# 10XGenomics/rust-pseudoaligner

Measured on AMD Instinct MI355X. Metric: reads/sec pseudoaligned (whole node) on synthetic 150bp reads, higher is better.
Workload: dtype u64; 1 GPU; config3: ~202k-transcript synthetic GENCODE-scale index (K=24), error-free 150bp reads; read_len=150, k=24, transcripts=201914, kmers=103866252, index_bytes=4833106924

## Files before the change

### rust-pseudoaligner_amd/csrc/map_pool.hip

```cpp
#include <hip/hip_runtime.h>

#include "kernels.hpp"
#include "lane_steps.hpp"
#include "kernel_utils.hpp"

#ifndef PA_FILL
#define PA_FILL 1
#endif
#ifndef PA_COOP_MIN
#define PA_COOP_MIN 2u
#endif
#ifndef PA_REFILL_ALIGN
#define PA_REFILL_ALIGN 1u
#endif
#ifndef PA_RARE_MIN
#define PA_RARE_MIN 16u
#endif

#ifdef PA_ISA_MARKS
#define PA_MARK(name) asm volatile("; PA_MARK " name ::: "memory")
#else
#define PA_MARK(name)
#endif

namespace pa {
namespace {

typedef __attribute__((address_space(3))) uint64_t* lds_u64;
typedef __attribute__((address_space(3))) uint32_t* lds_u32;
typedef __attribute__((address_space(3))) uint8_t* lds_u8;
typedef __attribute__((address_space(3))) uint16_t* lds_u16;
typedef __attribute__((address_space(3))) unsigned long long* lds_u64w;
typedef uint32_t u32x4 __attribute__((ext_vector_type(4)));
typedef __attribute__((address_space(3))) u32x4* lds_v4;
typedef __attribute__((address_space(1))) u32x4* glb_v4w;
typedef __attribute__((address_space(1))) const u32x4* glb_v4;
typedef __attribute__((address_space(1))) uint32_t* glb_u32w;
typedef __attribute__((address_space(1))) const uint32_t* glb_u32;
typedef __attribute__((address_space(1))) unsigned long long* glb_u64w;
__device__ __forceinline__ void store_result(glb_v4w dst, u32x4 v) {
    if (PA_NT & 2) __builtin_nontemporal_store(v, dst);
    else *dst = v;
}

typedef __attribute__((address_space(4))) const MapParams* karg_ptr;

__device__ __forceinline__ DevIndexView view_of(karg_ptr p) {
    DevIndexView v;
    v.table = p->ix.table; v.nbuckets = p->ix.nbuckets; v.blobs = p->ix.blobs; v.ledge = p->ix.ledge;
    v.seg_g = p->ix.seg_g; v.seg_nid = p->ix.seg_nid; v.ec = p->ix.ec; v.class_ref = p->ix.class_ref; v.class_len = p->ix.class_len;
    v.wtable = p->ix.wtable; v.wbuckets = p->ix.wbuckets; v.kmask = p->ix.kmask; v.kmask_hi = p->ix.kmask_hi; v.k = p->ix.k; v.num_nodes = p->ix.num_nodes; v.num_classes = p->ix.num_classes; v.num_segs = p->ix.num_segs; v.stream_nt = p->ix.stream_nt; v.bitmap_min = p->ix.bitmap_min; v.bitmap_words = p->ix.bitmap_words; v.dict_pairs = p->ix.dict_pairs;
    return v;
}

static_assert(ST_NSTAT == ST_COUNT + 4, "kernels.hpp");
constexpr uint32_t ST_DUAL = ST_COUNT;
constexpr uint32_t POOL_FIXED = 960;
constexpr uint32_t POOL_MAX_SLOTS = 128;
constexpr uint32_t LIST_ROW_HDR = 12;

__device__ __forceinline__ uint32_t rank_in(uint64_t m) { return __builtin_amdgcn_mbcnt_hi((uint32_t)(m >> 32), __builtin_amdgcn_mbcnt_lo((uint32_t)m, 0u)); }

__device__ __forceinline__ uint64_t shfl64(uint64_t v, uint32_t src) {
    return ((uint64_t)(uint32_t)__shfl((int)(v >> 32), (int)src, 64) << 32) | (uint32_t)__shfl((int)v, (int)src, 64);
}

__device__ __forceinline__ uint64_t arena_alloc(uint32_t cnt_alloc, uint32_t lane, karg_ptr p, lds_u64w chunk) {
    const uint32_t incl = wave_incl_scan(cnt_alloc);
    const uint32_t total = (uint32_t)__builtin_amdgcn_readlane((int)incl, 63);
    asm volatile("" ::: "memory");
    unsigned long long chunk_cur = chunk[0];
    if (total > 0) {
        if (chunk_cur + total > chunk[1]) {
            const unsigned long long want = total > PA_ARENA_CHUNK ? total : PA_ARENA_CHUNK;
            unsigned long long base = 0;
            if (lane == 0) base = atomicAdd(p->arena_top, want);
            base = ((unsigned long long)(uint32_t)__builtin_amdgcn_readfirstlane((int)(base >> 32)) << 32) | (uint32_t)__builtin_amdgcn_readfirstlane((int)base);
            chunk_cur = base;
            if (lane == 0) chunk[1] = base + want;
        }
        if (lane == 0) chunk[0] = chunk_cur + total;
    }
    asm volatile("" ::: "memory");
    return chunk_cur + (incl - cnt_alloc);
}

constexpr uint32_t NO_KEY = 0xFFFFFFFFu;
__device__ __forceinline__ void append_keys(uint32_t key, uint32_t lane, karg_ptr p, lds_u32 kchunk) {
    const uint64_t m = __ballot(key != NO_KEY);
    if (m == 0) return;
    const uint32_t cnt = (uint32_t)__popcll(m);
    const glb_u32w keys = (glb_u32w)p->keys;
    asm volatile("" ::: "memory");
    const uint32_t cur = kchunk[0], room = kchunk[1] - cur;
    uint32_t nbase = 0;
    if (cnt > room) {
        if (lane == 0) {
            nbase = (uint32_t)atomicAdd(p->keys_top, (unsigned long long)PA_KEY_CHUNK);
            if ((uint64_t)nbase + PA_KEY_CHUNK > p->keys_cap) { atomicOr(p->status, PA_STATUS_SPILL_OVERFLOW); nbase = 0; }
        }
        nbase = (uint32_t)__builtin_amdgcn_readfirstlane((int)nbase);
    }
    const uint32_t r = rank_in(m);
    if (key != NO_KEY) keys[r < room ? cur + r : nbase + (r - room)] = key;
    if (lane == 0) {
        if (cnt > room) { kchunk[0] = nbase + (cnt - room); kchunk[1] = nbase + PA_KEY_CHUNK; }
        else kchunk[0] = cur + cnt;
    }
    asm volatile("" ::: "memory");
}

__device__ __forceinline__ void append_deferred(bool has, u32x4 e0, u32x4 e1, uint32_t lane, karg_ptr p, lds_u32 dchunk) {
    const uint64_t m = __ballot(has);
    if (m == 0) return;
    const uint32_t cnt = (uint32_t)__popcll(m);
    const glb_v4w out = (glb_v4w)p->defer;
    asm volatile("" ::: "memory");
    const uint32_t cur = dchunk[0], room = dchunk[1] - cur;
    uint32_t nbase = 0;
    if (cnt > room) {
        if (lane == 0) {
            nbase = (uint32_t)atomicAdd(p->defer_top, (unsigned long long)PA_DEFER_CHUNK);
            if ((uint64_t)nbase + PA_DEFER_CHUNK > p->defer_cap) { atomicOr(p->status, PA_STATUS_SPILL_OVERFLOW); nbase = 0; }
        }
        nbase = (uint32_t)__builtin_amdgcn_readfirstlane((int)nbase);
    }
    if (has) {
        const uint32_t r = rank_in(m);
        const uint64_t at = 2ull * (r < room ? cur + r : nbase + (r - room));
        out[at] = e0;
        out[at + 1] = e1;
    }
    if (lane == 0) {
        if (cnt > room) { dchunk[0] = nbase + (cnt - room); dchunk[1] = nbase + PA_DEFER_CHUNK; }
        else dchunk[0] = cur + cnt;
    }
    asm volatile("" ::: "memory");
}

__device__ __forceinline__ uint32_t list_hits(glb_u32 ec, uint32_t xref, uint32_t nch, uint32_t maxch, const uint32_t (&b)[8]) {
    const glb_v4 xrec = (glb_v4)(ec + 4ull * xref);
    uint32_t acc = 0;
    for (uint32_t c0 = 0; c0 < maxch; c0 += 4) {
        u32x4 w[4];
#pragma unroll
        for (uint32_t t = 0; t < 4; ++t) w[t] = xrec[c0 + t < nch ? c0 + t : 0];
#pragma unroll
        for (uint32_t t = 0; t < 4; ++t)
            if (c0 + t < nch) {
                const U4 ww{w[t].x, w[t].y, w[t].z, w[t].w};
                acc |= scan_words(ww, c0 + t == 0, b);
            }
    }
    return acc;
}

__device__ __forceinline__ uint32_t wave_max(uint32_t v) {
    for (uint32_t o = 32; o; o >>= 1) v = max(v, (uint32_t)__shfl_xor((int)v, (int)o, 64));
    return (uint32_t)__builtin_amdgcn_readfirstlane((int)v);
}

__device__ __forceinline__ void window_hits(glb_u32 ec, uint32_t xref, uint32_t len, bool act, uint32_t b1, uint32_t b2, uint32_t bitmap_min, uint32_t& m1, uint32_t& m2) {
    const bool bm = act && bitmap_min != 0 && len >= bitmap_min;
    uint32_t bw[4] = {0u, 0u, 0u, 0u};
    if (__ballot(bm)) {
        if (bm) {
            const glb_u32 bits = ec + class_bitmap(xref, len);
            bw[0] = bits[b1 >> 5]; bw[1] = bits[(b1 >> 5) + 1]; bw[2] = bits[b2 >> 5]; bw[3] = bits[(b2 >> 5) + 1];
        }
    }
    act = act && !bm;
    const glb_v4 rec = (glb_v4)(ec + 4ull * xref);
    const uint32_t nch = act ? (len + 4) >> 2 : 0u;
    uint32_t c[2] = {0u, 0u}, e[2] = {nch, 0u};
    const bool lng = act && len > 64;
    if (__ballot(lng)) {
        if (lng) {
            const glb_u32 ids = ec + 4ull * xref + 1;
#pragma unroll
            for (uint32_t r = 0; r < 2; ++r) {
                const uint32_t b = r ? b2 : b1;
                uint32_t lo = 0, hi = len;
                while (lo < hi) {
                    const uint32_t mid = (lo + hi) >> 1;
                    if (ids[mid] < b) lo = mid + 1; else hi = mid;
                }
                c[r] = (1 + lo) >> 2;
                e[r] = min(nch, ((1 + lo + CLASS_WINDOW - 1) >> 2) + 1);
            }
        }
    }
    m1 = m2 = 0;
#pragma unroll
    for (uint32_t r = 0; r < 2; ++r) {
        const uint32_t mx = wave_max(e[r] > c[r] ? e[r] - c[r] : 0u);
        for (uint32_t c0 = 0; c0 < mx; c0 += 4) {
            u32x4 w[4];
#pragma unroll
            for (uint32_t t = 0; t < 4; ++t) w[t] = rec[c[r] + c0 + t < e[r] ? c[r] + c0 + t : 0u];
#pragma unroll
            for (uint32_t t = 0; t < 4; ++t)
                if (c[r] + c0 + t < e[r]) {
                    const uint32_t v[4] = {w[t].x, w[t].y, w[t].z, w[t].w};
#pragma unroll
                    for (uint32_t i = 0; i < 4; ++i) {
                        if (i == 0 && c[r] + c0 + t == 0) continue;
                        const uint32_t d1 = v[i] - b1, d2 = v[i] - b2;
                        if (d1 < CLASS_WINDOW) m1 |= 1u << d1;
                        if (d2 < CLASS_WINDOW) m2 |= 1u << d2;
                    }
                }
        }
    }
    if (bm) {
        m1 = (uint32_t)((((uint64_t)bw[1] << 32) | bw[0]) >> (b1 & 31u));
        m2 = (uint32_t)((((uint64_t)bw[3] << 32) | bw[2]) >> (b2 & 31u));
    }
}

}

namespace narrow {
#define PA_K_WIDE 0
#include "map_pool_kernel.inc"
#undef PA_K_WIDE
}

namespace wide {
#define PA_K_WIDE 1
#include "map_pool_kernel.inc"
#undef PA_K_WIDE
}

size_t pool_slot_bytes(uint32_t wpr) {
    return wpr > PA_LDS_READ_WORDS ? (size_t)wide::SLOT_FIXED_BYTES : 8 * (size_t)wpr + narrow::SLOT_FIXED_BYTES;
}
size_t pool_fixed_bytes() { return POOL_FIXED; }
uint32_t pool_max_slots() { return POOL_MAX_SLOTS; }

size_t pool_lds_bytes(uint32_t wpr, uint32_t slots) {
    const size_t wave_bytes = (POOL_FIXED + (size_t)slots * pool_slot_bytes(wpr) + 15) & ~(size_t)15;
    return wave_bytes * (PA_MAP_BLOCK / 64);
}

template <class K>
static int launch_kernel(K kernel, const MapParams& p, uint32_t grid, size_t lds_bytes, hipStream_t stream) {
    if (lds_bytes > 48 * 1024) {
        const hipError_t e = hipFuncSetAttribute(reinterpret_cast<const void*>(kernel), hipFuncAttributeMaxDynamicSharedMemorySize, (int)lds_bytes);
        if (e != hipSuccess) return (int)e;
    }
    hipLaunchKernelGGL(kernel, dim3(grid), dim3(PA_MAP_BLOCK), lds_bytes, stream, p);
    return (int)hipGetLastError();
}

int launch_map_pool(const MapParams& p, uint32_t grid, size_t lds_bytes, hipStream_t stream) {
    const bool gread = p.wpr > PA_LDS_READ_WORDS;
    const bool pair = p.ix.dict_pairs != 0;
    if (gread && pair) return p.trace ? launch_kernel(&wide::pa_map_pool_kernel<true, true, false, false, false, true>, p, grid, lds_bytes, stream)
                                      : launch_kernel(&wide::pa_map_pool_kernel<false, true, false, false, false, true>, p, grid, lds_bytes, stream);
    if (gread) return p.trace ? launch_kernel(&wide::pa_map_pool_kernel<true, true, false, false>, p, grid, lds_bytes, stream)
                              : launch_kernel(&wide::pa_map_pool_kernel<false, true, false, false>, p, grid, lds_bytes, stream);
    if (p.trace) return pair ? launch_kernel(&narrow::pa_map_pool_kernel<true, false, false, false, false, true>, p, grid, lds_bytes, stream)
                             : launch_kernel(&narrow::pa_map_pool_kernel<true, false, false, false>, p, grid, lds_bytes, stream);
#ifdef PA_DEBUG_KNOBS
    if (p.dbg || p.ablate) return pair ? launch_kernel(&narrow::pa_map_pool_kernel<false, false, true, false, false, true>, p, grid, lds_bytes, stream)
                                       : launch_kernel(&narrow::pa_map_pool_kernel<false, false, true, false>, p, grid, lds_bytes, stream);
#endif
    if (p.ix.k > 32)
        return p.pool_slots == 128 ? launch_kernel(&narrow::pa_map_pool_kernel<false, false, false, true, true>, p, grid, lds_bytes, stream)
                                   : launch_kernel(&narrow::pa_map_pool_kernel<false, false, false, false, true>, p, grid, lds_bytes, stream);
    if (pair) return p.pool_slots == 128 ? launch_kernel(&narrow::pa_map_pool_kernel<false, false, false, true, false, true>, p, grid, lds_bytes, stream)
                                         : launch_kernel(&narrow::pa_map_pool_kernel<false, false, false, false, false, true>, p, grid, lds_bytes, stream);
    if (p.pool_slots == 128) return launch_kernel(&narrow::pa_map_pool_kernel<false, false, false, true>, p, grid, lds_bytes, stream);
    return launch_kernel(&narrow::pa_map_pool_kernel<false, false, false, false>, p, grid, lds_bytes, stream);
}

int pool_kernel_occupancy(size_t lds_bytes, int* blocks_per_cu) {
    return (int)hipOccupancyMaxActiveBlocksPerMultiprocessor(blocks_per_cu, reinterpret_cast<const void*>(&narrow::pa_map_pool_kernel<false, false, false, false>),
                                                             PA_MAP_BLOCK, lds_bytes);
}

}
```

### rust-pseudoaligner_amd/csrc/map_pool_kernel.inc

```
namespace {

template <bool TRACE>
__device__ __forceinline__ void trace_out(const Lane& s, bool mapped, uint32_t gslot, karg_ptr p) {
    if (!TRACE) return;
    const uint32_t spill_cap = p->spill_cap;
    const uint32_t nt = l_ntrace(s);
    const uint32_t nn = mapped ? (nt < spill_cap ? nt : spill_cap) : 0;
    ((glb_u32w)p->nodes_len)[s.rid] = mapped ? nt : 0;
    const glb_u32w tr = (glb_u32w)p->trace + (uint64_t)gslot * spill_cap;
    const glb_u32w out = (glb_u32w)p->nodes_out + (uint64_t)s.rid * spill_cap;
    for (uint32_t j = 0; j < nn; ++j) out[j] = tr[j];
}

template <bool TRACE>
__device__ __forceinline__ uint32_t emit_record(Lane& s, uint32_t cnt, uint32_t cnt_alloc, uint64_t my_off, uint32_t base_len,
                                                uint32_t base_colour, uint32_t gslot, karg_ptr p, bool& defer) {
    uint32_t colour = NO_CLASS, class_off = (uint32_t)my_off;
    bool novel = false;
    if (my_off + cnt_alloc > p->arena_cap) atomicOr(p->status, PA_STATUS_ARENA_FULL);
    if (cnt == base_len) {
        colour = base_colour;
        class_off = PA_CLASS_REF | base_colour;
    } else novel = cnt != 0;
    if (l_flags(s) & F_SPILL_OVERFLOW) atomicOr(p->status, PA_STATUS_SPILL_OVERFLOW);
    ((glb_v4w)p->results)[s.rid] = u32x4{l_cov(s), l_mism(s) | PA_MAPPED_BIT, class_off, cnt};
    trace_out<TRACE>(s, true, gslot, p);
    const glb_u32w colour_out = (glb_u32w)p->colour_out;
    if (novel && (p->keys != nullptr || colour_out != nullptr) && my_off + cnt_alloc <= p->arena_cap) {
        defer = true;
        s.lk = 0;
        return NO_KEY;
    }
    if (colour_out) colour_out[s.rid] = colour;
    s.lk = 0;
    const uint32_t num_classes = p->ix.num_classes;
    return cnt == 0 ? num_classes + 1 : colour == NO_CLASS ? num_classes : colour;
}

__device__ __forceinline__ uint32_t queue_of(Lane& s, uint32_t K) {
    uint32_t st = l_st(s);
    if (st == ST_ISECT) {
        const uint32_t fl = l_flags(s);
        if (!(fl & F_LISTS)) {
            const uint32_t todo = window_todo(s);
            if (todo == 2) { restart_lists(s, K); return ST_SEEK; }
            st = todo ? ST_F_MASK : ST_F_BITS;
        } else st = l_ncol(s) <= 3 ? ST_F_LIGHT : (fl & F_SMALL_BASE) ? ST_F_SCAN : ST_F_COOP;
        l_set_st(s, st);
    }
    return st == ST_NONE ? (uint32_t)ST_F_BITS : st;
}

template <bool GREAD>
__device__ __forceinline__ void refill_slot(Lane& s, uint64_t rid, uint32_t slot, karg_ptr p, lds_u64 rd, lds_u32 wc, uint32_t S, uint32_t wpr,
                                            uint32_t K) {
    const uint32_t* lens = p->lens;
    uint32_t L = lens ? lens[rid] : p->uniform_len;
    if (L > wpr * 32) L = wpr * 32;
    if (!GREAD) {
        const uint64_t* src = p->tiles + ((rid >> 6) * wpr) * 64 + (rid & 63);
        if (wpr == 5) {
            const bool nt = (PA_NT & 1) || p->ix.stream_nt;
            const uint64_t v0 = ld_stream(src, nt), v1 = ld_stream(src + 64, nt), v2 = ld_stream(src + 128, nt), v3 = ld_stream(src + 192, nt), v4 = ld_stream(src + 256, nt);
            rd[slot] = v0; rd[S + slot] = v1; rd[2 * S + slot] = v2; rd[3 * S + slot] = v3; rd[4 * S + slot] = v4;
        } else if (wpr == 4) {
            const bool nt = (PA_NT & 1) || p->ix.stream_nt;
            const uint64_t v0 = ld_stream(src, nt), v1 = ld_stream(src + 64, nt), v2 = ld_stream(src + 128, nt), v3 = ld_stream(src + 192, nt);
            rd[slot] = v0; rd[S + slot] = v1; rd[2 * S + slot] = v2; rd[3 * S + slot] = v3;
        } else
        for (uint32_t w0 = 0; w0 < wpr; w0 += 8) {
            uint64_t v[8];
#pragma unroll
            for (uint32_t i = 0; i < 8; ++i) v[i] = w0 + i < wpr ? PA_LD(1, src + (uint64_t)(w0 + i) * 64) : 0ull;
#pragma unroll
            for (uint32_t i = 0; i < 8; ++i)
                if (w0 + i < wpr) rd[(w0 + i) * S + slot] = v[i];
        }
    }
    lane_start(s, (uint32_t)rid, L, K);
    wc[2 * slot + 1] = (uint32_t)rid;
}

__device__ __forceinline__ void lane_load(Lane& s, lds_v4 stA, lds_v4 stB, lds_v4 stC, uint32_t slot) {
    const u32x4 a = stA[slot], b = stB[slot];
    s.lk = a.x; s.cm = a.y; s.h = a.z; s.of = a.w; s.rr = b.x; s.rm = b.y; s.ph = b.z; s.nc = b.w;
#if PA_K_WIDE
    const u32x4 c = stC[slot];
    s.xl = c.x; s.xm = c.y; s.xt = c.z;
#else
    (void)stC;
#endif
}
__device__ __forceinline__ void lane_store(const Lane& s, lds_v4 stA, lds_v4 stB, lds_v4 stC, uint32_t slot) {
    stA[slot] = u32x4{s.lk, s.cm, s.h, s.of};
    stB[slot] = u32x4{s.rr, s.rm, s.ph, s.nc};
#if PA_K_WIDE
    stC[slot] = u32x4{s.xl, s.xm, s.xt, 0u};
#else
    (void)stC;
#endif
}
constexpr uint32_t SLOT_FIXED_BYTES = 32 + 16 + 8 + (PA_K_WIDE ? 16 : 0);

}

#ifndef PA_MAP_MIN_BLOCKS
#define PA_MAP_MIN_BLOCKS 3
#endif
template <bool TRACE, bool GREAD, bool DBG, bool S128 = false, bool KBIG = false, bool PAIR = false>
__global__ __launch_bounds__(PA_MAP_BLOCK, PA_MAP_MIN_BLOCKS) void pa_map_pool_kernel(const MapParams p_arg) {
    karg_ptr kp = (karg_ptr)__builtin_amdgcn_kernarg_segment_ptr();
    (void)p_arg;
#define p (*kp)
#define PA_DBG (DBG && p.dbg)
#define PA_ABLATE(bit) (DBG && (p.ablate & (bit)))
    extern __shared__ __attribute__((aligned(16))) uint8_t smem[];
    const uint32_t lane = lane_id();
    const uint32_t wave_in_block = (uint32_t)__builtin_amdgcn_readfirstlane((int)(threadIdx.x >> 6));
    const uint32_t waves_per_block = PA_MAP_BLOCK / 64;
    const uint32_t wave = blockIdx.x * waves_per_block + wave_in_block;
    const uint32_t nwaves = gridDim.x * waves_per_block;
    const uint32_t S = S128 ? 128u : p.pool_slots, wpr = p.wpr;
    const uint32_t lwpr = GREAD ? 0u : wpr;

    const uint32_t wave_bytes = (POOL_FIXED + S * (8 * lwpr + SLOT_FIXED_BYTES) + 15) & ~15u;
    uint8_t* const wbase = smem + wave_in_block * wave_bytes;
    const lds_u64w chunk = (lds_u64w)wbase;
    const lds_u32 dbg = (lds_u32)(wbase + 16);
    const lds_u64w dbg_clk = (lds_u64w)(wbase + 16 + 8 * ST_NSTAT);
    const lds_u32 kchunk = (lds_u32)(wbase + 256);
    const lds_u32 dchunk = (lds_u32)(wbase + 264);
    const lds_u64 rd = (lds_u64)(wbase + POOL_FIXED);
    const lds_v4 stA = (lds_v4)(wbase + POOL_FIXED + 8 * lwpr * S);
    const lds_v4 stB = (lds_v4)(wbase + POOL_FIXED + (8 * lwpr + 16) * S);
    constexpr uint32_t XW = PA_K_WIDE ? 16u : 0u;
    const lds_v4 stC = (lds_v4)(wbase + POOL_FIXED + (8 * lwpr + 32) * S);
    const lds_v4 win = (lds_v4)(wbase + POOL_FIXED + (8 * lwpr + 32 + XW) * S);
    const lds_u32 wc = (lds_u32)(wbase + POOL_FIXED + (8 * lwpr + 48 + XW) * S);
    const lds_u8 sb = (lds_u8)(wbase + 768);
    const lds_u8 poplist = (lds_u8)(wbase + 896);
    if (lane < 64) ((lds_u32)wbase)[lane] = 0;
    if (lane < 4) kchunk[lane] = 0;
    ((lds_u16)sb)[lane] = (uint16_t)((lane < S ? (uint32_t)ST_EMPTY : 0xFFu) | ((lane + 64 < S ? (uint32_t)ST_EMPTY : 0xFFu) << 8));

    const uint32_t ntiles = (uint32_t)((p.n_reads + 63) >> 6);
    const uint32_t chunk_tiles = ntiles / (nwaves * 4) >= 16 ? 16u : ntiles / (nwaves * 4) >= 1 ? ntiles / (nwaves * 4) : 1u;
    uint64_t next = (uint64_t)wave * chunk_tiles << 6;
    uint64_t end = (uint64_t)(wave + 1) * chunk_tiles << 6;
    if (end > p.n_reads) end = p.n_reads;
    if (next > end) next = end;
    bool more = true;
    uint32_t seen = nwaves * chunk_tiles;

    const bool counting = p.keys != nullptr;

#define PA_CNT(t) ((uint32_t)__popcll(__ballot(st_lo == (t))) + (uint32_t)__popcll(__ballot(st_hi == (t))))
#define PA_POP(t, nn, out)                                                                         \
    {                                                                                              \
        const uint64_t m0_ = __ballot(st_lo == (t)), m1_ = __ballot(st_hi == (t));                 \
        const uint32_t r1_ = (uint32_t)__popcll(m0_) + rank_in(m1_);                               \
        if (st_lo == (t)) poplist[rank_in(m0_)] = (uint8_t)lane;                                   \
        if (st_hi == (t) && r1_ < 64) poplist[r1_] = (uint8_t)(lane + 64);                         \
        asm volatile("" ::: "memory");                                                             \
        out = lane < (nn) ? (uint32_t)poplist[lane] : 0u;                                          \
        asm volatile("" ::: "memory");                                                             \
    }

    for (;;) {
        PA_MARK("loop_top");
        asm volatile("" : "+s"(kp) : : "memory");
        const DevIndexView ix = view_of(kp);
        const glb_u32 ec = (glb_u32)ix.ec;
        const uint32_t K = ix.k, allowed = p.allowed, spill_cap = p.spill_cap;
        if (next == end && more) {
            const uint32_t share = (ntiles > seen ? ntiles - seen : 0u) / (2 * nwaves);
            const uint32_t take = share >= 16 ? 16u : share >= 2 ? share : 2u;
            uint32_t t0 = 0;
            if (lane == 0) t0 = atomicAdd(p.tile_ctr, take);
            t0 = (uint32_t)__builtin_amdgcn_readfirstlane((int)t0) + nwaves * chunk_tiles;
            seen = t0 + take;
            if (t0 >= ntiles) more = false;
            else {
                next = (uint64_t)t0 << 6;
                end = (uint64_t)(t0 + take) << 6;
                if (end > p.n_reads) end = p.n_reads;
            }
        }
        const uint32_t st2 = (uint32_t)((lds_u16)sb)[lane];
        const uint32_t st_lo = st2 & 0xFFu, st_hi = st2 >> 8;
        const uint64_t left = end - next;
        const uint32_t nempty = PA_CNT(ST_EMPTY);
        const uint32_t nrefill = (uint32_t)(left < (uint64_t)nempty ? left : (uint64_t)nempty);
        uint32_t best = 0, sel = ST_EMPTY;
        uint32_t bestn = 0;
#define PA_CONSIDER(t, c) { const uint32_t c_ = (c); if (best < 64 && c_ > best) { best = c_; bestn = c_; sel = (t); } }
#define PA_CONSIDER_RARE_MIN(t, c, mn) { const uint32_t c_ = (c), w_ = (PA_RARE_MIN && c_ >= (mn)) ? 64u + c_ : c_; \
                                         if (best < 64 && w_ > best) { best = w_; bestn = c_; sel = (t); } }
#define PA_CONSIDER_RARE(t, c) PA_CONSIDER_RARE_MIN(t, c, PA_RARE_MIN)
        constexpr uint32_t RARE = (1u << ST_LEFT) | (1u << ST_F_LIGHT) | (1u << ST_F_SCAN) | (1u << ST_F_COOP) | (1u << ST_F_MASK);
        const bool any_rare = __ballot((((RARE >> (st_lo & 31u)) | (RARE >> (st_hi & 31u))) & 1u) != 0) != 0;
        const uint32_t n_bits_q = PA_CNT(ST_F_BITS), n_seek_q = PA_CNT(ST_SEEK), n_fwd_q = PA_CNT(ST_FWD);
        if (any_rare) {
            PA_CONSIDER_RARE_MIN(ST_F_COOP, PA_CNT(ST_F_COOP), PA_COOP_MIN)
            PA_CONSIDER_RARE(ST_F_SCAN, PA_CNT(ST_F_SCAN))
            PA_CONSIDER_RARE(ST_F_LIGHT, PA_CNT(ST_F_LIGHT))
            PA_CONSIDER_RARE(ST_F_MASK, PA_CNT(ST_F_MASK))
            PA_CONSIDER(ST_F_BITS, n_bits_q)
            PA_CONSIDER(ST_FWD, n_fwd_q)
            PA_CONSIDER_RARE(ST_LEFT, PA_CNT(ST_LEFT))
            PA_CONSIDER(ST_SEEK, n_seek_q)
            PA_CONSIDER(ST_EMPTY, nrefill)
        } else {
            const uint32_t cb = min(n_bits_q, 64u), cf = min(n_fwd_q, 64u), cs = min(n_seek_q, 64u), ce = min(nrefill, 64u);
            best = max(max(cb, cf), max(cs, ce));
            sel = cb == best ? (uint32_t)ST_F_BITS : cf == best ? (uint32_t)ST_FWD : cs == best ? (uint32_t)ST_SEEK : (uint32_t)ST_EMPTY;
            bestn = cb == best ? n_bits_q : cf == best ? n_fwd_q : cs == best ? n_seek_q : nrefill;
        }
#undef PA_CONSIDER
#undef PA_CONSIDER_RARE
#undef PA_CONSIDER_RARE_MIN
        if (best == 0) break;
#ifndef PA_SEEK_MIN
#define PA_SEEK_MIN 32u
#endif
        const bool seek_ok = n_seek_q >= PA_SEEK_MIN || n_fwd_q < 24;
        const bool dual = (sel == ST_FWD || sel == ST_SEEK) && (K <= 32 || KBIG) && n_seek_q != 0 && n_fwd_q != 0 && seek_ok && !PA_ABLATE(4u);
        if (dual) sel = ST_FWD;
        uint32_t n_own = dual ? (n_fwd_q < 64 ? n_fwd_q : 64) : bestn < 64 ? bestn : 64;
        if (PA_REFILL_ALIGN > 1 && sel == ST_EMPTY && n_own >= PA_REFILL_ALIGN && (uint64_t)n_own < left) n_own &= ~(PA_REFILL_ALIGN - 1u);
        const uint32_t n_fill = (PA_FILL && sel == ST_F_BITS && left != 0) ? (64 - n_own < nempty ? 64 - n_own : nempty) : 0u;
        const uint32_t n = n_own + n_fill;
        const uint32_t n2 = dual ? (n_seek_q < 64 ? n_seek_q : 64) : 0u;
        if (PA_DBG && lane == 0) {
            dbg[dual ? ST_DUAL : sel] += 1;
            dbg[ST_NSTAT + (dual ? ST_DUAL : sel)] += n + n2;
        }
        const unsigned long long t_sec = PA_DBG ? __builtin_readcyclecounter() : 0ull;

        PA_MARK("picked");
        const bool active = lane < n;
        uint32_t slot, slot2 = 0;
        PA_POP(sel, n_own, slot)
        if (n_fill) {
            uint32_t eslot;
            PA_POP((uint32_t)ST_EMPTY, n_fill, eslot)
            const uint32_t mine = (uint32_t)__shfl((int)eslot, (int)((lane - n_own) & 63u), 64);
            if (lane >= n_own && active) slot = mine;
        }
        const bool active2 = lane < n2;
        if (dual) PA_POP((uint32_t)ST_SEEK, n2, slot2)
        const uint32_t gslot = wave * S + slot;
        Lane s;
        {
            lane_load(s, stA, stB, stC, slot);
            s.rid = wc[2 * slot + 1];
            if (n_fill && lane >= n_own) s.lk = 0;
        }
        const ReadRef rr = GREAD ? ReadRef{p.tiles + ((uint64_t)(s.rid >> 6) * wpr) * 64 + (s.rid & 63), 64u, wpr} : ReadRef{(const uint64_t*)(rd + slot), S, wpr, true};
        const glb_u32w row = (glb_u32w)p.spill + (uint64_t)gslot * spill_cap;
        const ColRef cols{(uint32_t*)&win[slot], (uint32_t*)(wc + 2 * slot), (uint32_t*)row, (uint32_t*)(row + 4), (uint32_t*)(row + 8),
                          (uint32_t*)(row + LIST_ROW_HDR), spill_cap - LIST_ROW_HDR, (uint32_t*)row,
                          TRACE ? (uint32_t*)((glb_u32w)p.trace + (uint64_t)gslot * spill_cap) : nullptr};

        uint32_t nq2 = 0xFFu;
        PA_MARK("popped");
        const unsigned long long t_pop = PA_DBG ? __builtin_readcyclecounter() : 0ull;
        if (sel == ST_EMPTY) {
            if (active) refill_slot<GREAD>(s, next + lane, slot, kp, rd, wc, S, wpr, K);
            next += n;
        } else if (sel == ST_SEEK) {
            if (active) {
                if (PAIR) seek_step_pair(s, ix, rr);
                else seek_step_slots(s, ix, rr);
            }
        } else if (sel == ST_FWD) {
            __builtin_amdgcn_s_waitcnt(0x0F70);
            Lane s2;
            {
#if PA_K_WIDE
                lane_load(s2, stA, stB, stC, slot2);
                if (!active2) l_zero(s2);
#else
                const u32x4 a = stA[slot2], b = stB[slot2];
                s2.lk = active2 ? a.x : 0u; s2.cm = active2 ? a.y : 0u; s2.h = active2 ? a.z : 0u; s2.of = active2 ? a.w : 0u;
                s2.rr = active2 ? b.x : 0u; s2.rm = active2 ? b.y : 0u; s2.ph = active2 ? b.z : 0u; s2.nc = active2 ? b.w : 0u;
#endif
                s2.rid = 0;
            }
            if (!active) l_zero(s);
            const uint32_t rid2 = GREAD && active2 ? wc[2 * slot2 + 1] : 0u;
            const ReadRef rr2 = GREAD ? ReadRef{p.tiles + ((uint64_t)(rid2 >> 6) * wpr) * 64 + (rid2 & 63), 64u, wpr} : ReadRef{(const uint64_t*)(rd + slot2), S, wpr};
            SeekProbe pq;
            FwdLoad fl;
            PA_MARK("dual_state2");
            pq.klo = pq.khi = pq.pending = 0; pq.v = U4{0u, 0u, NO_HANDLE, 0u};
            SeekProbe2 pq2;
            if (KBIG) {
                pq2.k0 = pq2.v0 = pq2.k1 = pq2.v1 = U4{0u, 0u, 0u, 0u}; pq2.v0.x = pq2.v1.x = NO_HANDLE; pq2.w0 = pq2.w1 = pq2.w2 = pq2.w3 = 0;
                if (n2) seek_issue_k2(s2, ix, rr2, pq2);
            }
            if (PAIR && n2) seek_issue_pair(s2, ix, rr2, pq);
            if (!KBIG && !PAIR && n2) seek_issue(s2, ix, rr2, pq);
            const bool two_l = !KBIG && active2 && (PAIR ? seek_two_pair(s2, K) : seek_two(s2, K));
            const bool pairs = __popcll(__ballot(two_l)) >= 8;
            const bool two = two_l && pairs;
            SeekProbe pq1;
            pq1.klo = pq1.khi = pq1.pending = 0; pq1.v = U4{0u, 0u, NO_HANDLE, 0u};
            if (PAIR && pairs) seek_issue_pair(s2, ix, rr2, pq1, PA_SEEK_STRIDE, two);
            if (!PAIR && pairs) seek_issue(s2, ix, rr2, pq1, PA_SEEK_STRIDE, two);
            fwd_issue(s, ix, fl);
            __builtin_amdgcn_sched_barrier(0);
            PA_MARK("dual_issued");
            if (active2) {
                if (KBIG) seek_complete_k2(s2, K, pq2);
                else if (PAIR) seek_complete2_pair(s2, K, pq, two, pq1);
                else seek_complete2(s2, K, pq, two, pq1);
                nq2 = queue_of(s2, K);
                lane_store(s2, stA, stB, stC, slot2);
            }
            __builtin_amdgcn_sched_barrier(0);
            const unsigned long long t1 = PA_DBG ? __builtin_readcyclecounter() : 0ull;
            PA_MARK("dual_second");
            if (active) fwd_finish<TRACE>(s, ix, rr, cols, allowed, fl);
            PA_MARK("dual_fwd_done");
            if (PA_DBG && lane == 0) {
                const unsigned long long t3 = __builtin_readcyclecounter();
                dbg[ST_COUNT + 1] += 1; dbg[ST_COUNT + 3] += 1;
                dbg_clk[ST_COUNT + 1] += t1 - t_pop; dbg_clk[ST_COUNT + 3] += t3 - t1;
            }
            PA_MARK("dual_seek_done");
        } else if (sel == ST_LEFT) {
            if (active) left_step<TRACE>(s, ix, rr, cols, allowed);
        } else if (sel == ST_F_BITS) {
            PA_MARK("bits_begin");
            uint32_t ckey = NO_KEY;
            bool dfr = false;
            u32x4 d0{0u, 0u, 0u, 0u}, d1{0u, 0u, 0u, 0u};
            if (active && lane < n_own) {
                const bool mapped = l_st(s) != ST_NONE;
                const u32x4 w = win[slot];
                const uint32_t cand = wc[2 * slot];
                const uint32_t count = mapped ? (uint32_t)(__popc(w.y) + __popc(w.w)) : 0u;
                if (mapped && count != 0 && cand == NO_CLASS) {
                    dfr = true;
                    d0 = u32x4{s.rid, l_cov(s), l_mism(s), PA_DEFER_WINDOW | count};
                    d1 = w;
                    trace_out<TRACE>(s, true, gslot, kp);
                    s.lk = 0;
                } else {
                    const bool is_ref = mapped && count != 0;
                    if (!PA_ABLATE(1u))
                        store_result((glb_v4w)p.results + s.rid, mapped ? u32x4{l_cov(s), l_mism(s) | PA_MAPPED_BIT, is_ref ? PA_CLASS_REF | cand : 0u, count}
                                                                        : u32x4{0u, 0u, 0u, 0u});
                    trace_out<TRACE>(s, mapped, gslot, kp);
                    const glb_u32w colour_out = (glb_u32w)p.colour_out;
                    if (colour_out) colour_out[s.rid] = is_ref ? cand : NO_CLASS;
                    ckey = !mapped ? ix.num_classes + 2 : count == 0 ? ix.num_classes + 1 : cand;
                    s.lk = 0;
                }
            }
            {
                const uint64_t freed = __ballot(active && s.lk == 0);
                const uint32_t nfree = (uint32_t)__popcll(freed);
                uint32_t take = (uint32_t)(left < (uint64_t)nfree ? left : (uint64_t)nfree);
                if (PA_REFILL_ALIGN > 1 && take >= PA_REFILL_ALIGN && (uint64_t)take < left) take &= ~(PA_REFILL_ALIGN - 1u);
                if (take && !PA_ABLATE(8u)) {
                    if (active && s.lk == 0 && rank_in(freed) < take) refill_slot<GREAD>(s, next + rank_in(freed), slot, kp, rd, wc, S, wpr, K);
                    next += take;
                }
            }
            if (counting && !PA_ABLATE(2u)) append_keys(ckey, lane, kp, kchunk);
            append_deferred(dfr, d0, d1, lane, kp, dchunk);
            PA_MARK("bits_end");
        } else if (sel == ST_F_MASK) {
            const u32x4 w = active ? win[slot] : u32x4{0u, 0u, 0u, 0u};
            const uint32_t np_mine = active ? l_npend(s) : 0u;
            uint32_t a1 = w.y, a2 = w.w;
            for (uint64_t todo = __ballot(active && np_mine <= 64); todo;) {
                const uint32_t want = ((todo >> lane) & 1ull) ? np_mine : 0u;
                const uint32_t incl = wave_incl_scan(want);
                const uint32_t start = incl - want;
                const bool inpass = want != 0 && incl <= 64;
                const uint64_t pass = __ballot(inpass);
                todo &= ~pass;
                uint32_t Lr = 64, jg = 0, seg_end = 0;
                for (uint64_t m = pass; m; m &= m - 1) {
                    const uint32_t o = (uint32_t)(__ffsll((unsigned long long)m) - 1);
                    const uint32_t st = (uint32_t)__builtin_amdgcn_readlane((int)start, (int)o);
                    const uint32_t nc = (uint32_t)__builtin_amdgcn_readlane((int)np_mine, (int)o);
                    if (lane - st < nc) { Lr = o; jg = lane - st; seg_end = st + nc; }
                }
                const bool gact = Lr < 64;
                const int src = (int)(Lr & 63u);
                const uint32_t b1 = (uint32_t)__shfl((int)w.x, src, 64), b2 = (uint32_t)__shfl((int)w.z, src, 64), slotL = (uint32_t)__shfl((int)slot, src, 64);
                const glb_u32w rowL = (glb_u32w)p.spill + (uint64_t)(wave * S + slotL) * spill_cap;
                uint32_t xref = 0, xlen = 0;
                if (gact) { xref = rowL[2 * jg]; xlen = rowL[2 * jg + 1]; }
                uint32_t m1, m2;
                window_hits(ec, xref, xlen, gact, b1, b2, ix.bitmap_min, m1, m2);
                for (uint32_t o = 1; o < 64; o <<= 1) {
                    const uint32_t t1 = (uint32_t)__shfl_down((int)m1, o, 64), t2 = (uint32_t)__shfl_down((int)m2, o, 64);
                    if (gact && lane + o < seg_end) { m1 &= t1; m2 &= t2; }
                }
                const uint32_t r1 = (uint32_t)__shfl((int)m1, (int)(start & 63u), 64), r2 = (uint32_t)__shfl((int)m2, (int)(start & 63u), 64);
                if (inpass) { a1 &= r1; a2 &= r2; }
            }
            for (uint64_t todo = __ballot(active && np_mine > 64); todo; todo &= todo - 1) {
                const uint32_t Lr = (uint32_t)(__ffsll((unsigned long long)todo) - 1);
                const uint32_t b1 = (uint32_t)__shfl((int)w.x, (int)Lr, 64), b2 = (uint32_t)__shfl((int)w.z, (int)Lr, 64);
                const uint32_t npL = (uint32_t)__shfl((int)np_mine, (int)Lr, 64), slotL = (uint32_t)__shfl((int)slot, (int)Lr, 64);
                const glb_u32w rowL = (glb_u32w)p.spill + (uint64_t)(wave * S + slotL) * spill_cap;
                uint32_t r1 = 0xFFFFFFFFu, r2 = 0xFFFFFFFFu;
                for (uint32_t g = 0; g < npL; g += 64) {
                    const uint32_t ci = g + lane;
                    const bool gact = ci < npL;
                    uint32_t xref = 0, xlen = 0;
                    if (gact) { xref = rowL[2 * ci]; xlen = rowL[2 * ci + 1]; }
                    uint32_t m1, m2;
                    window_hits(ec, xref, xlen, gact, b1, b2, ix.bitmap_min, m1, m2);
                    if (gact) { r1 &= m1; r2 &= m2; }
                }
                for (uint32_t o = 32; o; o >>= 1) {
                    r1 &= (uint32_t)__shfl_xor((int)r1, (int)o, 64);
                    r2 &= (uint32_t)__shfl_xor((int)r2, (int)o, 64);
                }
                if (lane == Lr) { a1 &= r1; a2 &= r2; }
            }
            if (active) {
                if (a1 != w.y || a2 != w.w) wc[2 * slot] = NO_CLASS;
                win[slot] = u32x4{w.x, a1, w.z, a2};
                s.nc = (s.nc & ~NC_COL_MASK) | 1u;
                l_set_st(s, ST_F_BITS);
            }
        } else if (sel == ST_F_SCAN) {
            Isect is;
            is.base_len = is.base_ref = is.base_colour = 0;
            if (active) isect_pick(s, cols, is);
            const uint32_t ncol_mine = l_ncol(s);
            if (active && ncol_mine > 3) is.base_colour = ec[4ull * is.base_ref];
            uint32_t my_alive = 0;
            for (uint64_t todo = __ballot(active && ncol_mine > 0 && ncol_mine <= 64); todo;) {
                const uint32_t want = ((todo >> lane) & 1ull) ? ncol_mine : 0u;
                const uint32_t incl = wave_incl_scan(want);
                const uint32_t start = incl - want;
                const bool inpass = want != 0 && incl <= 64;
                const uint64_t pass = __ballot(inpass);
                todo &= ~pass;
                uint32_t Lr = 64, jg = 0;
                for (uint64_t m = pass; m; m &= m - 1) {
                    const uint32_t o = (uint32_t)(__ffsll((unsigned long long)m) - 1);
                    const uint32_t st = (uint32_t)__builtin_amdgcn_readlane((int)start, (int)o);
                    const uint32_t nc = (uint32_t)__builtin_amdgcn_readlane((int)ncol_mine, (int)o);
                    if (lane - st < nc) { Lr = o; jg = lane - st; }
                }
                const bool gact = Lr < 64;
                const int src = (int)(Lr & 63u);
                const uint32_t bref = (uint32_t)__shfl((int)is.base_ref, src, 64), blen = (uint32_t)__shfl((int)is.base_len, src, 64),
                               slotL = (uint32_t)__shfl((int)slot, src, 64);
                const glb_u32w rowL = (glb_u32w)p.spill + (uint64_t)(wave * S + slotL) * spill_cap;
                const glb_v4 brec = (glb_v4)(ec + 4ull * bref);
                const u32x4 q0 = brec[0], q1 = brec[1], q2 = brec[2];
                const uint32_t b[8] = {q0.y, q0.z, q0.w, q1.x, q1.y, q1.z, q1.w, blen > 7 ? q2.x : 0xFFFFFFFFu};
                uint32_t xref = bref, xlen = 0;
                if (gact) {
                    if (jg < LDS_CLASSES) { xref = rowL[jg]; xlen = rowL[4 + jg]; }
                    else { const u32x4 qd = *(glb_v4)(rowL + LIST_ROW_HDR + 4 * (jg - LDS_CLASSES)); xref = qd.x; xlen = qd.y; }
                }
                const bool mine = xref != bref;
                const uint32_t nch = mine ? (xlen + 4) >> 2 : 0u;
                uint32_t maxch = nch;
                for (uint32_t o = 32; o; o >>= 1) maxch = max(maxch, (uint32_t)__shfl_xor((int)maxch, (int)o, 64));
                maxch = (uint32_t)__builtin_amdgcn_readfirstlane((int)maxch);
                const uint32_t acc = list_hits(ec, xref, nch, maxch, b);
                const uint32_t miss = mine ? ~acc & 0xFFu : 0u;
                const uint64_t seg = inpass ? (want == 64 ? ~0ull : ((1ull << want) - 1) << start) : 0ull;
                uint32_t alive = (1u << is.base_len) - 1;
#pragma unroll
                for (uint32_t kk = 0; kk < 8; ++kk)
                    if (__ballot((miss >> kk) & 1u) & seg) alive &= ~(1u << kk);
                if (inpass) my_alive = alive;
            }
            for (uint64_t todo = __ballot(active && ncol_mine > 64); todo; todo &= todo - 1) {
                const uint32_t Lr = (uint32_t)(__ffsll((unsigned long long)todo) - 1);
                const uint32_t bref = (uint32_t)__shfl((int)is.base_ref, (int)Lr, 64);
                const uint32_t blen = (uint32_t)__shfl((int)is.base_len, (int)Lr, 64);
                const uint32_t ncolL = (uint32_t)__shfl((int)ncol_mine, (int)Lr, 64);
                const uint32_t slotL = (uint32_t)__shfl((int)slot, (int)Lr, 64);
                const glb_u32w rowL = (glb_u32w)p.spill + (uint64_t)(wave * S + slotL) * spill_cap;
                const glb_v4 brec = (glb_v4)(ec + 4ull * bref);
                const u32x4 q0 = brec[0], q1 = brec[1], q2 = brec[2];
                const uint32_t b[8] = {q0.y, q0.z, q0.w, q1.x, q1.y, q1.z, q1.w, blen > 7 ? q2.x : 0xFFFFFFFFu};
                uint32_t alive = (1u << blen) - 1;
                for (uint32_t g = 0; g < ncolL && alive; g += 64) {
                    const uint32_t ci = g + lane;
                    uint32_t xref = bref, xlen = 0;
                    if (ci < ncolL) {
                        if (ci < LDS_CLASSES) { xref = rowL[ci]; xlen = rowL[4 + ci]; }
                        else { const u32x4 qd = *(glb_v4)(rowL + LIST_ROW_HDR + 4 * (ci - LDS_CLASSES)); xref = qd.x; xlen = qd.y; }
                    }
                    const bool mine = xref != bref;
                    const uint32_t nch = mine ? (xlen + 4) >> 2 : 0u;
                    uint32_t maxch = nch;
                    for (uint32_t o = 32; o; o >>= 1) maxch = max(maxch, (uint32_t)__shfl_xor((int)maxch, (int)o, 64));
                    maxch = (uint32_t)__builtin_amdgcn_readfirstlane((int)maxch);
                    const uint32_t acc = list_hits(ec, xref, nch, maxch, b);
#pragma unroll
                    for (uint32_t kk = 0; kk < 8; ++kk)
                        if (__ballot(mine && !((acc >> kk) & 1u))) alive &= ~(1u << kk);
                }
                if (lane == Lr) my_alive = alive;
            }
            const uint32_t cnt = active ? (uint32_t)__popc(my_alive) : 0u;
            const uint32_t cnt_alloc = active && cnt != is.base_len ? cnt : 0u;
            const uint64_t my_off = arena_alloc(cnt_alloc, lane, kp, chunk);
            uint32_t ckey = NO_KEY;
            bool dfr = false;
            u32x4 d0{0u, 0u, 0u, 0u}, d1{0u, 0u, 0u, 0u};
            if (active) {
                if (cnt_alloc && my_off + cnt_alloc <= p.arena_cap) {
                    const glb_u32w dst = (glb_u32w)p.arena + my_off;
                    const glb_u32 bids = ec + 4ull * is.base_ref + 1;
                    uint32_t k = 0;
                    for (uint32_t t = my_alive; t; t &= t - 1) dst[k++] = bids[__ffs((int)t) - 1];
                }
                const uint32_t cov_ = l_cov(s), mm_ = l_mism(s);
                ckey = emit_record<TRACE>(s, cnt, cnt_alloc, my_off, is.base_len, is.base_colour, gslot, kp, dfr);
                d0 = u32x4{s.rid, cov_, mm_, PA_DEFER_LIST | cnt};
                d1 = u32x4{(uint32_t)my_off, 0u, 0u, 0u};
            }
            if (counting) append_keys(ckey, lane, kp, kchunk);
            append_deferred(dfr, d0, d1, lane, kp, dchunk);
        } else if (sel == ST_F_COOP) {
            Isect is;
            is.count = 0;
            is.base_len = is.base_ref = is.base_colour = 0;
            if (active) isect_pick(s, cols, is);
            if (active && l_ncol(s) > 3) is.base_colour = ec[4ull * is.base_ref];
            const uint32_t cnt_alloc = active ? is.base_len : 0u;
            const uint64_t my_off = arena_alloc(cnt_alloc, lane, kp, chunk);
            const uint64_t arena_cap = p.arena_cap;
            const glb_u32w arena_g = (glb_u32w)p.arena;
            const uint32_t ncol_mine = l_ncol(s);
            uint32_t my_count = 0;
            for (uint32_t Lr = 0; Lr < n; ++Lr) {
                const uint32_t bref = (uint32_t)__shfl((int)is.base_ref, (int)Lr, 64);
                const uint32_t blen = (uint32_t)__shfl((int)is.base_len, (int)Lr, 64);
                const uint32_t ncolL = (uint32_t)__shfl((int)ncol_mine, (int)Lr, 64);
                const uint32_t slotL = (uint32_t)__shfl((int)slot, (int)Lr, 64);
                const uint64_t off = shfl64(my_off, Lr);
                const bool fits = off + blen <= arena_cap;
                const glb_u32w rowL = (glb_u32w)p.spill + (uint64_t)(wave * S + slotL) * spill_cap;
                uint32_t total = 0;
                uint32_t cref = 0, clen = 0;
                if (lane < ncolL) {
                    const glb_u32w e = lane < LDS_CLASSES ? rowL + lane : rowL + LIST_ROW_HDR + 4 * (lane - LDS_CLASSES);
                    cref = e[0];
                    clen = lane < LDS_CLASSES ? e[4] : e[1];
                }
                for (uint32_t c = 0; c < blen; c += 64) {
                    const uint32_t j = c + lane;
                    const bool valid = j < blen;
                    const uint32_t v = valid ? ec[4ull * bref + 1 + j] : 0u;
                    bool ok = valid;
                    for (uint32_t i = 0; i < ncolL; ++i) {
                        uint32_t ref, len;
                        if (i < 64) {
                            ref = (uint32_t)__shfl((int)cref, (int)i, 64);
                            len = (uint32_t)__shfl((int)clen, (int)i, 64);
                        } else {
                            const glb_u32w e = rowL + LIST_ROW_HDR + 4 * (i - LDS_CLASSES);
                            ref = e[0];
                            len = e[1];
                        }
                        if (ref == bref) continue;
                        bool hit = false;
                        if (len <= 64) {
                            const glb_v4 rec = (glb_v4)(ec + 4ull * ref);
                            const uint32_t nchunks = (len + 4) >> 2;
                            for (uint32_t q0 = 0; q0 < nchunks; q0 += 4) {
                                u32x4 x[4];
#pragma unroll
                                for (uint32_t t = 0; t < 4; ++t) x[t] = rec[q0 + t < nchunks ? q0 + t : q0];
#pragma unroll
                                for (uint32_t t = 0; t < 4; ++t)
                                    if (q0 + t < nchunks) hit |= (q0 + t != 0 && x[t].x == v) | (x[t].y == v) | (x[t].z == v) | (x[t].w == v);
                            }
                        } else {
                            const glb_u32 ids = ec + 4ull * ref + 1;
                            uint32_t lo = 0, hi = len;
                            while (lo < hi) {
                                const uint32_t mid = (lo + hi) >> 1;
                                if (ids[mid] < v) lo = mid + 1; else hi = mid;
                            }
                            hit = lo < len && ids[lo] == v;
                        }
                        ok = ok && hit;
                    }
                    const uint64_t bm = __ballot(ok);
                    if (ok && fits) arena_g[off + total + rank_in(bm)] = v;
                    total += (uint32_t)__popcll(bm);
                }
                if (lane == Lr) my_count = total;
            }
            uint32_t ckey = NO_KEY;
            bool dfr = false;
            u32x4 d0{0u, 0u, 0u, 0u}, d1{0u, 0u, 0u, 0u};
            if (active) {
                const uint32_t cov_ = l_cov(s), mm_ = l_mism(s);
                ckey = emit_record<TRACE>(s, my_count, cnt_alloc, my_off, is.base_len, is.base_colour, gslot, kp, dfr);
                d0 = u32x4{s.rid, cov_, mm_, PA_DEFER_LIST | my_count};
                d1 = u32x4{(uint32_t)my_off, 0u, 0u, 0u};
            }
            if (counting) append_keys(ckey, lane, kp, kchunk);
            append_deferred(dfr, d0, d1, lane, kp, dchunk);
        } else {
            Isect is;
            is.count = 0;
            is.base_len = 0xFFFFFFFFu;
            is.base_ref = is.base_colour = 0;
            is.alive = 0;
            is.in_regs = false;
#pragma unroll
            for (int j = 0; j < 7; ++j) is.ids[j] = 0;
            bool emit_now = active;
            if (active) {
                const uint32_t tier = isect_pick(s, cols, is);
                if (tier == 0) isect_light(s, ix, cols, is);
                else {
                    l_set_st(s, tier == 1 ? ST_F_SCAN : ST_F_COOP);
                    emit_now = false;
                }
            }
            const uint32_t cntv2 = emit_now ? is.count : 0u;
            const uint32_t cnt_alloc = cntv2 == is.base_len ? 0u : cntv2;
            const uint64_t my_off = arena_alloc(cnt_alloc, lane, kp, chunk);
            uint32_t ckey = NO_KEY;
            bool dfr = false;
            u32x4 d0{0u, 0u, 0u, 0u}, d1{0u, 0u, 0u, 0u};
            if (emit_now) {
                if (cnt_alloc && my_off + cnt_alloc <= p.arena_cap) {
                    const glb_u32w dst = (glb_u32w)p.arena + my_off;
                    const uint32_t alive = (uint32_t)is.alive;
#pragma unroll
                    for (int j = 0; j < 7; ++j)
                        if ((alive >> j) & 1u) dst[__popc(alive & ((1u << j) - 1))] = is.ids[j];
                }
                const uint32_t cov_ = l_cov(s), mm_ = l_mism(s);
                ckey = emit_record<TRACE>(s, cntv2, cnt_alloc, my_off, is.base_len, is.base_colour, gslot, kp, dfr);
                d0 = u32x4{s.rid, cov_, mm_, PA_DEFER_LIST | cntv2};
                d1 = u32x4{(uint32_t)my_off, 0u, 0u, 0u};
            }
            if (counting) append_keys(ckey, lane, kp, kchunk);
            append_deferred(dfr, d0, d1, lane, kp, dchunk);
        }

        const unsigned long long t_step = PA_DBG ? __builtin_readcyclecounter() : 0ull;
        PA_MARK("step_done");
        const uint32_t nq = active ? queue_of(s, K) : 0xFFu;
        if (active) lane_store(s, stA, stB, stC, slot);
        if (active) sb[2 * (slot & 63u) + (slot >> 6)] = (uint8_t)nq;
        if (active2) sb[2 * (slot2 & 63u) + (slot2 >> 6)] = (uint8_t)nq2;
        if (PA_DBG && lane == 0) {
            const unsigned long long t_end = __builtin_readcyclecounter();
            dbg_clk[dual ? ST_DUAL : sel] += t_end - t_sec;
            dbg[ST_ISECT] += 1;
            dbg_clk[ST_ISECT] += t_pop - t_sec;
            dbg[ST_NONE] += 1;
            dbg_clk[ST_NONE] += t_end - t_step;
        }
        PA_MARK("stored");
    }
    {
        asm volatile("" ::: "memory");
        const uint32_t cur = dchunk[0], end = dchunk[1];
        for (uint32_t i = cur + lane; i < end; i += 64) ((glb_v4w)p.defer)[2ull * i] = u32x4{NO_KEY, 0u, 0u, 0u};
    }
    if (counting) {
        asm volatile("" ::: "memory");
        const uint32_t cur = kchunk[0], end = kchunk[1];
        for (uint32_t i = cur + lane; i < end; i += 64) ((glb_u32w)p.keys)[i] = NO_KEY;
    }
    if (PA_DBG && lane < 2 * ST_NSTAT) atomicAdd(p.dbg + lane, (unsigned long long)dbg[lane]);
    if (PA_DBG && lane < ST_NSTAT) atomicAdd(p.dbg + 2 * ST_NSTAT + lane, dbg_clk[lane]);
#undef PA_CNT
#undef PA_POP
#undef PA_DBG
#undef PA_ABLATE
#undef p
}
```

Baseline: 13.85 billion reads/s.

## Issue first seek probe at refill time and favor full seek batches

When lanes are refilled with new reads, the first seek probe into the index is issued right away. In the bits path, that probe overlaps with the key and deferred-record appends before it is settled. The scheduler is also changed to prefer seek steps once at least PA_SEEK_FULL lanes are waiting, and to lower the seek threshold for dual mode. The aim is to hide the index-lookup latency of fresh reads and cut the number of scheduler iterations. In exchange it adds work and register pressure to the refill paths and changes the state scheduling balance.

```diff
diff --git a/rust-pseudoaligner_amd/csrc/map_pool.hip b/rust-pseudoaligner_amd/csrc/map_pool.hip
--- a/rust-pseudoaligner_amd/csrc/map_pool.hip
+++ b/rust-pseudoaligner_amd/csrc/map_pool.hip
@@ -12,6 +12,15 @@
 #endif
 #ifndef PA_REFILL_ALIGN
 #define PA_REFILL_ALIGN 1u
+#endif
+#ifndef PA_SEEK_MIN
+#define PA_SEEK_MIN 32u
+#endif
+#ifndef PA_PROBE_AT_REFILL
+#define PA_PROBE_AT_REFILL 1
+#endif
+#ifndef PA_SEEK_FULL
+#define PA_SEEK_FULL 8u
 #endif
 #ifndef PA_RARE_MIN
 #define PA_RARE_MIN 16u
diff --git a/rust-pseudoaligner_amd/csrc/map_pool_kernel.inc b/rust-pseudoaligner_amd/csrc/map_pool_kernel.inc
--- a/rust-pseudoaligner_amd/csrc/map_pool_kernel.inc
+++ b/rust-pseudoaligner_amd/csrc/map_pool_kernel.inc
@@ -81,6 +81,22 @@
     wc[2 * slot + 1] = (uint32_t)rid;
 }
 
+template <bool PAIR>
+__device__ __forceinline__ bool fresh_probe_issue(const Lane& s, bool fresh, const DevIndexView& ix, ReadRef rr, SeekProbe& q) {
+    const bool live = fresh && l_st(s) == ST_SEEK && (PAIR || ix.k <= 32);
+    Lane t = s;
+    if (!live) l_zero(t);
+    if (PAIR) seek_issue_pair(t, ix, rr, q, 0, live);
+    else seek_issue(t, ix, rr, q, 0, live);
+    return live;
+}
+template <bool PAIR>
+__device__ __forceinline__ void fresh_probe_settle(Lane& s, bool live, uint32_t K, const SeekProbe& q) {
+    if (!live) return;
+    if (PAIR) (void)seek_settle_pair(s, K, q, false);
+    else (void)seek_settle(s, K, q, false);
+}
+
 __device__ __forceinline__ void lane_load(Lane& s, lds_v4 stA, lds_v4 stB, lds_v4 stC, uint32_t slot) {
     const u32x4 a = stA[slot], b = stB[slot];
     s.lk = a.x; s.cm = a.y; s.h = a.z; s.of = a.w; s.rr = b.x; s.rm = b.y; s.ph = b.z; s.nc = b.w;
@@ -172,6 +188,7 @@
         const DevIndexView ix = view_of(kp);
         const glb_u32 ec = (glb_u32)ix.ec;
         const uint32_t K = ix.k, allowed = p.allowed, spill_cap = p.spill_cap;
+        constexpr bool par = PA_PROBE_AT_REFILL && !GREAD && !KBIG;
         if (next == end && more) {
             const uint32_t share = (ntiles > seen ? ntiles - seen : 0u) / (2 * nwaves);
             const uint32_t take = share >= 16 ? 16u : share >= 2 ? share : 2u;
@@ -200,6 +217,8 @@
         constexpr uint32_t RARE = (1u << ST_LEFT) | (1u << ST_F_LIGHT) | (1u << ST_F_SCAN) | (1u << ST_F_COOP) | (1u << ST_F_MASK);
         const bool any_rare = __ballot((((RARE >> (st_lo & 31u)) | (RARE >> (st_hi & 31u))) & 1u) != 0) != 0;
         const uint32_t n_bits_q = PA_CNT(ST_F_BITS), n_seek_q = PA_CNT(ST_SEEK), n_fwd_q = PA_CNT(ST_FWD);
+        const uint32_t seek_min = par && PA_SEEK_FULL ? PA_SEEK_FULL : PA_SEEK_MIN;
+        const uint32_t seek_w = par && PA_SEEK_FULL && n_seek_q >= PA_SEEK_FULL ? 64u + n_seek_q : n_seek_q;
         if (any_rare) {
             PA_CONSIDER_RARE_MIN(ST_F_COOP, PA_CNT(ST_F_COOP), PA_COOP_MIN)
             PA_CONSIDER_RARE(ST_F_SCAN, PA_CNT(ST_F_SCAN))
@@ -208,10 +227,10 @@
             PA_CONSIDER(ST_F_BITS, n_bits_q)
             PA_CONSIDER(ST_FWD, n_fwd_q)
             PA_CONSIDER_RARE(ST_LEFT, PA_CNT(ST_LEFT))
-            PA_CONSIDER(ST_SEEK, n_seek_q)
+            if (best < 64 && seek_w > best) { best = seek_w; bestn = n_seek_q; sel = ST_SEEK; }
             PA_CONSIDER(ST_EMPTY, nrefill)
         } else {
-            const uint32_t cb = min(n_bits_q, 64u), cf = min(n_fwd_q, 64u), cs = min(n_seek_q, 64u), ce = min(nrefill, 64u);
+            const uint32_t cb = min(n_bits_q, 64u), cf = min(n_fwd_q, 64u), cs = min(seek_w, 64u), ce = min(nrefill, 64u);
             best = max(max(cb, cf), max(cs, ce));
             sel = cb == best ? (uint32_t)ST_F_BITS : cf == best ? (uint32_t)ST_FWD : cs == best ? (uint32_t)ST_SEEK : (uint32_t)ST_EMPTY;
             bestn = cb == best ? n_bits_q : cf == best ? n_fwd_q : cs == best ? n_seek_q : nrefill;
@@ -220,10 +239,7 @@
 #undef PA_CONSIDER_RARE
 #undef PA_CONSIDER_RARE_MIN
         if (best == 0) break;
-#ifndef PA_SEEK_MIN
-#define PA_SEEK_MIN 32u
-#endif
-        const bool seek_ok = n_seek_q >= PA_SEEK_MIN || n_fwd_q < 24;
+        const bool seek_ok = n_seek_q >= seek_min || n_fwd_q < 24;
         const bool dual = (sel == ST_FWD || sel == ST_SEEK) && (K <= 32 || KBIG) && n_seek_q != 0 && n_fwd_q != 0 && seek_ok && !PA_ABLATE(4u);
         if (dual) sel = ST_FWD;
         uint32_t n_own = dual ? (n_fwd_q < 64 ? n_fwd_q : 64) : bestn < 64 ? bestn : 64;
@@ -268,6 +284,11 @@
         if (sel == ST_EMPTY) {
             if (active) refill_slot<GREAD>(s, next + lane, slot, kp, rd, wc, S, wpr, K);
             next += n;
+            if (par) {
+                SeekProbe pq;
+                const bool live = fresh_probe_issue<PAIR>(s, active, ix, rr, pq);
+                fresh_probe_settle<PAIR>(s, live, K, pq);
+            }
         } else if (sel == ST_SEEK) {
             if (active) {
                 if (PAIR) seek_step_pair(s, ix, rr);
@@ -359,18 +380,24 @@
                     s.lk = 0;
                 }
             }
+            bool fresh = false;
             {
                 const uint64_t freed = __ballot(active && s.lk == 0);
                 const uint32_t nfree = (uint32_t)__popcll(freed);
                 uint32_t take = (uint32_t)(left < (uint64_t)nfree ? left : (uint64_t)nfree);
                 if (PA_REFILL_ALIGN > 1 && take >= PA_REFILL_ALIGN && (uint64_t)take < left) take &= ~(PA_REFILL_ALIGN - 1u);
                 if (take && !PA_ABLATE(8u)) {
-                    if (active && s.lk == 0 && rank_in(freed) < take) refill_slot<GREAD>(s, next + rank_in(freed), slot, kp, rd, wc, S, wpr, K);
+                    fresh = active && s.lk == 0 && rank_in(freed) < take;
+                    if (fresh) refill_slot<GREAD>(s, next + rank_in(freed), slot, kp, rd, wc, S, wpr, K);
                     next += take;
                 }
             }
+            SeekProbe pq;
+            bool live = false;
+            if (par) live = fresh_probe_issue<PAIR>(s, fresh, ix, rr, pq);
             if (counting && !PA_ABLATE(2u)) append_keys(ckey, lane, kp, kchunk);
             append_deferred(dfr, d0, d1, lane, kp, dchunk);
+            if (par) fresh_probe_settle<PAIR>(s, live, K, pq);
             PA_MARK("bits_end");
         } else if (sel == ST_F_MASK) {
             const u32x4 w = active ? win[slot] : u32x4{0u, 0u, 0u, 0u};
```

New measurement: 14.30 billion reads/s (median of 6 runs). 1.03x the previous value.
